# nessex/rdst

Measured on AMD Instinct MI355X. Metric: radix_sort_throughput_1B_uniform_u32, higher is better.
Workload: dtype u32; 1 GPU; 1000000000 uniform-random u32 keys per GPU, device-resident; route 'atomic': two MSD scatter passes that claim space with atomics (no counting read) + in-LDS sort of every bucket; keys_per_gpu=1000000000, total_keys=1000000000, seed=1565982722, route=atomic, parallelism=single

## Files before the change

### rdst_amd/csrc/rdst_kernels.hip

```cpp

#include <hip/hip_runtime.h>
#include <stdint.h>
#include <string.h>
#include <stdio.h>
#include <stdlib.h>
#include <stddef.h>
#include <mutex>
#include <type_traits>
#include <string>
#include <vector>
#include <map>
#include <utility>

#include "rdst_hip.h"
#include "rdst_internal.h"

namespace {

constexpr int RADIX = 256;
constexpr int MAX_LEVELS = 16;

constexpr uint32_t ST_EMPTY = 0, ST_AGG = 1, ST_INCL = 2;
template <typename S> struct StatusWord {
    static constexpr int SHIFT = sizeof(S) * 8 - 2;
// ... 1395 lines not shown
        if constexpr (STAGES > 1) {
            if (stage > 0) __syncthreads();
#pragma unroll
            for (int i = 0; i < KPT; ++i) {
                const uint32_t sl = (i & 1) ? (slots[i >> 1] >> 16) : (slots[i >> 1] & 0xFFFFu);
                const uint32_t rel = sl - (uint32_t)(stage * STAGE_KEYS);
                if (rel < (uint32_t)STAGE_KEYS) s_keys[rel] = mk[i];
            }
            __syncthreads();
        }
        constexpr int SUB = SPT % 6 == 0 ? 6 : (SPT % 4 == 0 ? 4 : (SPT < 6 ? SPT : 6));
#pragma unroll
        for (int i0 = 0; i0 < SPT; i0 += SUB) {
            K kk[SUB];
            D dd[SUB];
            V vv[HAS_V ? SUB : 1];
#pragma unroll
            for (int i = 0; i < SUB; ++i)
                if (i0 + i < SPT) kk[i] = s_keys[tid + (i0 + i) * BLOCK];
            if constexpr (HAS_V) {
#pragma unroll
                for (int i = 0; i < SUB; ++i)
                    if (i0 + i < SPT) vv[i] = s_vals[tid + (i0 + i) * BLOCK];
            }
#pragma unroll
            for (int i = 0; i < SUB; ++i)
                if (i0 + i < SPT) dd[i] = s_delta[digit_of(kk[i], shift)];
#pragma unroll
            for (int i = 0; i < SUB; ++i) {
                if (i0 + i >= SPT) continue;
                const uint32_t p = (uint32_t)(stage * STAGE_KEYS) + (uint32_t)tid + (uint32_t)(i0 + i) * BLOCK;
                K out = kk[i];
                if constexpr (MAPPED) out = unmap_key<K>(out, neg, pos);
                if (RDST_ABL(1) && out != (K)0x12345) continue;
                if (RDST_ABL(2)) {
                    if (full || p < valid) dst[tile_begin + p] = out;
                    continue;
                }
                if constexpr (NARROW) {
                    const uint32_t g = dd[i] + p * (uint32_t)sizeof(K);
                    const bool ok = g < (uint32_t)n * (uint32_t)sizeof(K);
                    bad |= !ok && (full || p < valid);
                    if constexpr (OUT16) {
                        if (halves) {
                            if (ok && (full || p < valid)) *reinterpret_cast<uint16_t*>(reinterpret_cast<unsigned char*>(out16) + (g >> 1)) = (uint16_t)kk[i];
                            continue;
                        }
                    }
                    if (ok && (full || p < valid)) {
                        *reinterpret_cast<K*>(reinterpret_cast<unsigned char*>(dst) + g) = out;
                        if constexpr (HAS_V) {
                            const uint32_t gv = sizeof(V) == sizeof(K) ? g : (sizeof(V) > sizeof(K) ? g * (uint32_t)(sizeof(V) / sizeof(K)) : g / (uint32_t)(sizeof(K) / sizeof(V)));
                            *reinterpret_cast<V*>(reinterpret_cast<unsigned char*>(vdst) + gv) = vv[i];
                        }
                    }
                } else {
                    const uint64_t g = dd[i] + p;
                    const bool ok = g < n;
                    bad |= !ok && (full || p < valid);
                    if (ok && (full || p < valid)) {
                        dst[g] = out;
                        if constexpr (HAS_V) vdst[g] = vv[i];
                    }
                }
            }
        }
    }
    if (bad) atomicOr(err, ERR_SCATTER_RANGE | ((uint32_t)(level + 1) << 8));
#ifdef RDST_EXPERIMENTS
    RDST_STAMP(9);
    if (tl_on) {
        uint32_t* rec = g_exp_timeline + (size_t)(chain_row0 + t) * 12;
        for (int k = 0; k < 10; ++k) rec[k] = tl[k];
        rec[10] = __builtin_amdgcn_s_getreg(20 | (0 << 6) | (3 << 11));
        rec[11] = blockIdx.x;
    }
#endif
    if constexpr (!PERSIST) break;
    __syncthreads();
    }
#undef RDST_ABL
}

struct MsdRanges {
    uint64_t start[CHAINS + 1];
};

template <typename K, int KPT, int NWAVES, bool MAPPED, bool SECOND, bool HALVES>
#ifndef RDST_MSD_MINWAVES
#define RDST_MSD_MINWAVES ((2 * NWAVES + 3) / 4)
#endif
__global__ __launch_bounds__(NWAVES * 64, RDST_MSD_MINWAVES) void msd_scatter_kernel(
    const K* __restrict__ src, const uint32_t* __restrict__ area_count , uint64_t n, uint32_t area_cap,
    uint32_t tiles_per_area, K* __restrict__ dst, uint16_t* __restrict__ dst16, uint32_t* __restrict__ cursor, uint32_t dst_cap, int shift,
    uint32_t slices ,
    const Plan* __restrict__ plan, uint32_t* __restrict__ overflow, uint32_t* __restrict__ inversion ,
    K neg, K pos,
    K* __restrict__ xbuf, K* __restrict__ xout, const uint32_t* __restrict__ bstart, const uint32_t* __restrict__ xtile0,
    MsdRanges xr) {
    static_assert(!HALVES || (SECOND && sizeof(K) == 4), "halves: the second pass of 4-byte keys");
    constexpr int BLOCK = NWAVES * 64, TILE = BLOCK * KPT;
    constexpr uint32_t SLOT_UNIT = (uint32_t)sizeof(K);
    const bool exact = plan->pre != 0;
    if (exact) {
        if (plan->route != ROUTE_HYBRID || plan->sorted_known) return;
        if (!SECOND && plan->pre_skip_a) return;
    } else {
        if (plan->gross_skew || plan->top_skew || plan->predict_lsd) return;
        if (SECOND && *inversion == 0) return;
    }
    const int win = exact ? 0 : (int)plan->win_shift;
    shift -= win;
    extern __shared__ __attribute__((aligned(16))) unsigned char smem[];
    uint32_t* wave_hist = reinterpret_cast<uint32_t*>(smem);
    uint32_t* s_delta = reinterpret_cast<uint32_t*>(smem + NWAVES * 1024);
    uint32_t* s_misc = reinterpret_cast<uint32_t*>(smem + NWAVES * 1024 + 1024);
    K* s_keys = reinterpret_cast<K*>(smem + NWAVES * 1024 + 1024 + 128);
    const int tid = threadIdx.x, lane = tid & 63, wave = tid >> 6;
    static_assert(NWAVES <= 16, "one word of s_misc per wave");
    uint32_t gave_up = 0;
    if (!exact) {
        gave_up = ld_relaxed<uint32_t>(overflow);
        if constexpr (!SECOND) {
            if (gave_up) {
                if (lane == 0) s_misc[16 + wave] = 1u;
                __syncthreads();
                return;
            }
        }
    }
    uint32_t area = blockIdx.x / tiles_per_area, j = blockIdx.x % tiles_per_area;
    if constexpr (SECOND) {
        if (!exact && slices == (uint32_t)CHAINS) {
            const uint32_t x = blockIdx.x % CHAINS, k = blockIdx.x / CHAINS;
            const uint32_t q = k / tiles_per_area;
            j = k % tiles_per_area;
            area = (q % CHAINS) * RADIX + (x + CHAINS * (q / CHAINS));
        }
        if (!exact && (blockIdx.x / tiles_per_area >= RADIX * slices || area >= RADIX * slices)) return;
    }
    uint64_t acount = area_count ? (uint64_t)area_count[area] : n;
    const K* asrc = src + (uint64_t)area * area_cap;
    if (exact) {
        if constexpr (!SECOND) {
            area = blockIdx.x % CHAINS; j = blockIdx.x / CHAINS;
            acount = xr.start[area + 1] - xr.start[area];
            asrc = src + xr.start[area];
        } else {
            if (blockIdx.x >= xtile0[RADIX]) return;
            uint32_t d = 0;
#pragma unroll
            for (int b = 7; b >= 0; --b) {
                const uint32_t c = d | (1u << b);
                if (xtile0[c] <= blockIdx.x) d = c;
            }
            area = d; j = blockIdx.x - xtile0[d];
            const uint32_t r0 = bstart[d * RADIX];
            acount = bstart[(d + 1) * RADIX] - r0;
            asrc = (plan->pre_skip_a ? static_cast<const K*>(xout) : static_cast<const K*>(xbuf)) + r0;
        }
    }
    const uint64_t tile_off = (uint64_t)j * TILE;
    if (tile_off >= acount) return;
    const uint32_t valid = acount - tile_off < (uint64_t)TILE ? (uint32_t)(acount - tile_off) : (uint32_t)TILE;
    const bool full = valid == (uint32_t)TILE;
    const K* tsrc = asrc + tile_off;
    RDST_TL_BEGIN(SECOND ? 3u : 2u);
    __builtin_amdgcn_s_setprio(RDST_PRIO_LOAD);
    K mk[KPT];
    const uint32_t wbase = (uint32_t)wave * 64u * KPT + (uint32_t)lane;
    K edge = 0;
    if constexpr (!SECOND) {
        if (lane == 0 && tile_off + (uint64_t)wave * 64u * KPT > 0 && (uint32_t)wave * 64u * KPT < valid) edge = tsrc[(int64_t)wbase - 1];
    }
    if (full) {
#pragma unroll
        for (int i = 0; i < KPT; ++i) mk[i] = tsrc[wbase + i * 64];
        if constexpr (MAPPED) {
#pragma unroll
            for (int i = 0; i < KPT; ++i) mk[i] = map_key<K>(mk[i], neg, pos);
        }
    } else {
#pragma unroll
        for (int i = 0; i < KPT; ++i) {
            const uint32_t idx = wbase + i * 64;
            K v = (K)~(K)0;
            if (idx < valid) {
                v = tsrc[idx];
                if constexpr (MAPPED) v = map_key<K>(v, neg, pos);
            }
            mk[i] = v;
        }
    }
    if constexpr (!SECOND) if (!exact) {
        if constexpr (MAPPED) edge = map_key<K>(edge, neg, pos);
        if (tile_off + (uint64_t)wave * 64u * KPT == 0) edge = 0;
        bool inv = false;
#pragma unroll
        for (int i = 0; i < KPT; ++i) {
            K before = lane_below<K>(mk[i]);
// ... 72 lines not shown
                        ranked = true;
                    }
                    run3[h] += (uint32_t)__builtin_popcountll(m);
                }
                if (!ranked) r = atomicAdd(&wh[d], 1u);
                if (i & 1) run_index[i >> 1] |= r << 16;
                else run_index[i >> 1] = r;
            }
#pragma unroll
            for (int h = 0; h < NHEAVY; ++h)
                if (lane == 0 && hd3[h] != 0xFFFFFFFFu) wh[hd3[h]] = run3[h];
        } else if (fast) {
#pragma unroll
            for (int i = 0; i < KPT; ++i) {
                const uint32_t r = atomicAdd(&wh[digit_of(mk[i], shift)], 1u);
                if (i & 1) run_index[i >> 1] |= r << 16;
                else run_index[i >> 1] = r;
            }
        } else {
#pragma unroll
            for (int i = 0; i < KPT; ++i) atomicAdd(&wh[digit_of(mk[i], shift)], 1u);
        }
    }
    RDST_STAMP(2);
    if (lane == 0) s_misc[16 + wave] = gave_up;
    __syncthreads();
    {
        uint32_t any = 0;
#pragma unroll
        for (int w = 0; w < NWAVES; ++w) any |= s_misc[16 + w];
        if (any) return;
    }
    RDST_STAMP(3);
    if (tid < RADIX) __builtin_amdgcn_s_setprio(RDST_PRIO_SCAN);
    uint32_t cw[NWAVES];
    uint32_t count_d = 0, pub = 0;
    if (tid < RADIX) {
#pragma unroll
        for (int w = 0; w < NWAVES; ++w) {
            cw[w] = wave_hist[w * RADIX + tid];
            count_d += cw[w];
        }
        pub = count_d;
        if (tid == RADIX - 1) pub -= (uint32_t)TILE - valid;
    }
    uint32_t incl = count_d;
#pragma unroll
    for (int o = 1; o < 64; o <<= 1) {
        const uint32_t y = __shfl_up(incl, o);
        if (lane >= o) incl += y;
    }
    if (tid < RADIX && lane == 63) s_misc[4 + wave] = incl;
    if (tid == 0) s_misc[1] = 0;
    __syncthreads();
    if (tid < RADIX) {
        uint32_t woff = 0;
        for (int w = 0; w < wave; ++w) woff += s_misc[4 + w];
        const uint32_t local_off = woff + incl - count_d;
        uint32_t run = local_off;
#pragma unroll
        for (int w = 0; w < NWAVES; ++w) {
            wave_hist[w * RADIX + tid] = run * SLOT_UNIT;
            run += cw[w];
        }
        const uint32_t where = SECOND ? (area % RADIX) * RADIX + (uint32_t)tid : (exact ? area : blockIdx.x % slices) * RADIX + (uint32_t)tid;
        uint32_t got = 0;
        if (pub) {
            got = atomicAdd(&cursor[where], pub);
            if (!exact && got + pub > dst_cap) {
                if (ld_relaxed<uint32_t>(overflow) == 0) atomicOr(overflow, 1u);
                s_misc[1] = 1;
            }
        }
        s_delta[tid] = (exact ? 0u : where * dst_cap) + got - local_off;
    }
    RDST_STAMP(4);
    __syncthreads();
    RDST_STAMP(5);
    __builtin_amdgcn_s_setprio(0);
    if (fast) {
#pragma unroll
        for (int i = 0; i < KPT; ++i) {
            const uint32_t idx = (i & 1) ? (run_index[i >> 1] >> 16) : (run_index[i >> 1] & 0xFFFFu);
            const uint32_t sl = wh[digit_of(mk[i], shift)] + idx * SLOT_UNIT;
            *reinterpret_cast<K*>(reinterpret_cast<unsigned char*>(s_keys) + sl) = mk[i];
        }
    } else if (!careful) {
#pragma unroll
        for (int i = 0; i < KPT; ++i) {
            uint32_t* slot = &wh[digit_of(mk[i], shift)];
            const uint32_t b = *slot;
            const uint32_t below = peers_below(digit_word<K>(mk[i], shift), bit0);
            __builtin_amdgcn_wave_barrier();
            atomicAdd(slot, SLOT_UNIT);
            *reinterpret_cast<K*>(reinterpret_cast<unsigned char*>(s_keys) + b + below * SLOT_UNIT) = mk[i];
        }
    } else {
#pragma unroll
        for (int i = 0; i < KPT; ++i) {
            uint32_t* slot = &wh[digit_of(mk[i], shift)];
            const uint32_t b = *slot;
            uint32_t below;
            if ((uniform_rounds >> i) & 1u) {
                below = (uint32_t)lane;
                __builtin_amdgcn_wave_barrier();
                if (lane == 0) *slot = b + 64u * SLOT_UNIT;
            } else {
                uint32_t total;
                below = peers_below_total(digit_word<K>(mk[i], shift), bit0, total);
                __builtin_amdgcn_wave_barrier();
                if (below == 0) *slot = b + total * SLOT_UNIT;
            }
            *reinterpret_cast<K*>(reinterpret_cast<unsigned char*>(s_keys) + b + below * SLOT_UNIT) = mk[i];
        }
    }
    RDST_STAMP(6);
    __syncthreads();
    RDST_STAMP(7);
    if (s_misc[1]) return;
    __builtin_amdgcn_s_setprio(RDST_PRIO_SCATTER);
    constexpr int SUB = KPT % 6 == 0 ? 6 : (KPT % 4 == 0 ? 4 : (KPT < 6 ? KPT : 6));
#pragma unroll
    for (int i0 = 0; i0 < KPT; i0 += SUB) {
        K kk[SUB];
        uint32_t dd[SUB];
#pragma unroll
        for (int i = 0; i < SUB; ++i)
            if (i0 + i < KPT) kk[i] = s_keys[tid + (i0 + i) * BLOCK];
#pragma unroll
        for (int i = 0; i < SUB; ++i)
            if (i0 + i < KPT) dd[i] = s_delta[digit_of(kk[i], shift)];
#pragma unroll
        for (int i = 0; i < SUB; ++i) {
            if (i0 + i >= KPT) continue;
            const uint32_t p = (uint32_t)tid + (uint32_t)(i0 + i) * BLOCK;
            if (full || p < valid) {
                const uint32_t g = dd[i] + p;
                if constexpr (HALVES) dst16[g] = (uint16_t)kk[i];
                else (exact ? (SECOND ? xout : xbuf) : dst)[g] = MAPPED ? unmap_key<K>(kk[i], neg, pos) : kk[i];
            }
        }
    }
    RDST_STAMP(8);
    RDST_TL_END(blockIdx.x);
}

constexpr int SMALL_WAVES = 16;
constexpr int SMALL_THREADS = SMALL_WAVES * 64;
constexpr int small_kpt(size_t key_bytes) { return key_bytes <= 4 ? 16 : (key_bytes == 8 ? 8 : 4); }

template <typename K, int LEVELS, bool MAPPED>
__global__ __launch_bounds__(SMALL_THREADS) void small_sort_kernel(K* __restrict__ keys, uint32_t n, K neg, K pos) {
    constexpr int KPT = small_kpt(sizeof(K));
    constexpr int TILE = SMALL_THREADS * KPT;
    extern __shared__ __attribute__((aligned(16))) unsigned char smem[];
    uint32_t* wave_hist = reinterpret_cast<uint32_t*>(smem);
    uint32_t* s_sum = reinterpret_cast<uint32_t*>(smem + SMALL_WAVES * 1024);
    K* stage = reinterpret_cast<K*>(smem + SMALL_WAVES * 1024 + 16);
    const int tid = threadIdx.x, lane = tid & 63, wave = tid >> 6;
    const int rounds = (int)((n + SMALL_THREADS - 1) / SMALL_THREADS);
    const uint32_t live = (uint32_t)rounds * SMALL_THREADS;
    const uint32_t wbase = (uint32_t)wave * 64u * (uint32_t)rounds + (uint32_t)lane;
    K mk[KPT];
#pragma unroll
    for (int i = 0; i < KPT; ++i) {
        const uint32_t idx = wbase + i * 64;
        K v = (K) ~(K)0;
        if (i < rounds && idx < n) {
            v = keys[idx];
            if constexpr (MAPPED) v = map_key<K>(v, neg, pos);
        }
        mk[i] = v;
    }
    uint32_t* wh = wave_hist + wave * RADIX;
    for (int level = 0; level < LEVELS; ++level) {
        const int shift = level * 8, bit0 = shift & 31;
#pragma unroll
        for (int j = 0; j < 4; ++j) wh[lane + 64 * j] = 0;
#pragma unroll
        for (int i = 0; i < KPT; ++i)
            if (i < rounds) atomicAdd(&wh[digit_of(mk[i], shift)], 1u);
        __syncthreads();
        uint32_t cw[SMALL_WAVES], count_d = 0;
        if (tid < RADIX) {
#pragma unroll
            for (int w = 0; w < SMALL_WAVES; ++w) { cw[w] = wave_hist[w * RADIX + tid]; count_d += cw[w]; }
        }
        const bool trivial = __syncthreads_or(tid < RADIX && count_d == live) != 0;
        if (trivial) continue;
        uint32_t incl = count_d;
#pragma unroll
        for (int o = 1; o < 64; o <<= 1) {
            const uint32_t y = __shfl_up(incl, o);
            if (lane >= o) incl += y;
        }
        if (tid < RADIX && lane == 63) s_sum[wave] = incl;
        __syncthreads();
        if (tid < RADIX) {
            uint32_t run = incl - count_d;
            for (int w = 0; w < wave; ++w) run += s_sum[w];
#pragma unroll
            for (int w = 0; w < SMALL_WAVES; ++w) { wave_hist[w * RADIX + tid] = run; run += cw[w]; }
        }
        __syncthreads();
#pragma unroll
        for (int i = 0; i < KPT; ++i) {
            if (i < rounds) {
                uint32_t* slot = &wh[digit_of(mk[i], shift)];
                const uint32_t b = *slot;
                const uint32_t below = peers_below(digit_word<K>(mk[i], shift), bit0);
                __builtin_amdgcn_wave_barrier();
                atomicAdd(slot, 1u);
                stage[b + below] = mk[i];
            }
// ... 243 lines not shown
        local_sort_bucket<K, NWAVES, KPT, MAPPED>(buf, src16, alt_src, slot_count ? bucket * slot_cap : start, bucket, bucket_prefix16(plan, bucket), start, cnt, err, neg, pos, flags);
        __syncthreads();
    }
}

constexpr int COUNT_TILE = local_tile(4);
constexpr size_t count_lds_bytes() { return 32768 + 16384 + 128; }
static_assert(2 * ((size_t)COUNT_TILE + 4) <= 32768 + 16384, "the output staging (shifted by up to three keys) aliases the counter and prefix tables");

__device__ __forceinline__ uint32_t nibble_sum(uint32_t x, uint32_t acc) {
    const uint32_t t = (x & 0x0F0F0F0Fu) + ((x >> 4) & 0x0F0F0F0Fu);
    return __builtin_amdgcn_sad_u8(t, 0u, acc);
}

constexpr int COUNT_SAFE = 24;

template <int BLOCK, bool MAPPED, bool FROM16, bool FAST, bool VEC>
__device__ __forceinline__ void count_sort_bucket(uint32_t* __restrict__ buf, const uint16_t* __restrict__ src16, uint32_t soff, uint32_t start, uint32_t cnt,
                                                  uint32_t bucket, const Plan* __restrict__ plan, uint32_t neg, uint32_t pos, uint32_t* __restrict__ list,
                                                  uint32_t* __restrict__ list_count, unsigned char* smem) {
    constexpr int MAXR = (COUNT_TILE + BLOCK - 1) / BLOCK;
    constexpr int VPT = H16_BINS / BLOCK, WPT = VPT / 8;
    constexpr int LOG_VPT = BLOCK == 1024 ? 6 : (BLOCK == 512 ? 7 : 8);
    static_assert((1 << LOG_VPT) == VPT, "block size");
    static_assert(!VEC || (FROM16 && MAXR == 33 && BLOCK == 512), "vector loads: four vectors of eight halves and one half per thread");
    static_assert(COUNT_SAFE % 8 == 0 && COUNT_SAFE < MAXR, "whole vectors");
    const int tid = threadIdx.x, lane = tid & 63, wave = tid >> 6;
    uint32_t* cnt4 = reinterpret_cast<uint32_t*>(smem);
    uint16_t* prefix = reinterpret_cast<uint16_t*>(smem + 32768);
    uint16_t* out16 = reinterpret_cast<uint16_t*>(smem);
    uint32_t* s_wsum = reinterpret_cast<uint32_t*>(smem + 32768 + 16384);
    auto idx_of = [&](int i) -> uint32_t {
        if constexpr (VEC) return i < 32 ? 8u * ((uint32_t)tid + (uint32_t)(i >> 3) * BLOCK) + (uint32_t)(i & 7) : 32u * BLOCK + (uint32_t)tid;
        else return (uint32_t)tid + (uint32_t)i * BLOCK;
    };
    uint32_t nvalid = 0;
    if constexpr (VEC) {
#pragma unroll
        for (int j = 0; j < 4; ++j) {
            const uint32_t v0 = 8u * ((uint32_t)tid + (uint32_t)j * BLOCK);
            nvalid += cnt > v0 ? (cnt - v0 < 8u ? cnt - v0 : 8u) : 0u;
        }
        nvalid += 32u * BLOCK + (uint32_t)tid < cnt ? 1u : 0u;
    } else {
        nvalid = cnt > (uint32_t)tid ? (cnt - (uint32_t)tid + BLOCK - 1u) / BLOCK : 0u;
    }
#define RDST_K4_PHASE() uint32_t nv_ = nvalid; asm volatile("" : "+v"(nv_))
#define RDST_K4_VALID(i) ((FAST && (i) < COUNT_SAFE) || (uint32_t)(i) < nv_)
#define RDST_K4_FENCE(i) do { if (((i) & 3) == 3 || (i) == MAXR - 1) { _Pragma("unroll") for (int f_ = (i) - ((i) & 3); f_ <= (i); ++f_) asm volatile("" : "+v"(kv[f_])); } } while (0)
#define RDST_K4_OPAQUE() do { _Pragma("unroll") for (int i_ = 0; i_ < MAXR; ++i_) asm volatile("" : "+v"(kv[i_])); } while (0)
    __builtin_amdgcn_s_setprio(RDST_PRIO_LOAD);
    uint32_t kv[MAXR];
    if constexpr (VEC) {
        const uint4* vsrc = reinterpret_cast<const uint4*>(src16 + soff);
        uint4 q[4];
#pragma unroll
        for (int j = 0; j < 4; ++j) {
            const uint32_t vi = (uint32_t)tid + j * BLOCK;
            if ((FAST && j < COUNT_SAFE / 8) || 8u * vi < cnt) q[j] = vsrc[vi];
            else q[j] = make_uint4(0, 0, 0, 0);
        }
        kv[32] = 32u * BLOCK + (uint32_t)tid < cnt ? (uint32_t)src16[soff + 32u * BLOCK + (uint32_t)tid] : 0u;
#pragma unroll
        for (int j = 0; j < 4; ++j) {
            const uint32_t d[4] = {q[j].x, q[j].y, q[j].z, q[j].w};
#pragma unroll
            for (int e = 0; e < 4; ++e) {
                kv[8 * j + 2 * e] = d[e] & 0xFFFFu;
                kv[8 * j + 2 * e + 1] = d[e] >> 16;
            }
        }
    } else {
        RDST_K4_PHASE();
#pragma unroll
        for (int i = 0; i < MAXR; ++i) {
            const uint32_t idx = idx_of(i);
            const uint32_t at = RDST_K4_VALID(i) ? idx : cnt - 1;
            if constexpr (FROM16) kv[i] = src16[soff + at];
            else kv[i] = buf[start + at];
        }
    }
#pragma unroll
    for (int k = 0; k < WPT; ++k) cnt4[k * BLOCK + tid] = 0;
    if (tid == 0) s_wsum[16] = 0;
    __syncthreads();
    __builtin_amdgcn_s_setprio(0);
    auto word_of = [](uint32_t v) -> uint32_t { return v >> 3; };
    bool over = false;
    {
    RDST_K4_PHASE();
#pragma unroll
    for (int i = 0; i < MAXR; ++i) {
        if (RDST_K4_VALID(i)) {
            const uint32_t v = FROM16 ? kv[i] : ((MAPPED ? map_key<uint32_t>(kv[i], neg, pos) : kv[i]) & 0xFFFFu);
            const uint32_t sh = (v & 7u) * 4u;
            const uint32_t old = atomicAdd(&cnt4[word_of(v)], 1u << sh);
            const uint32_t mine = (old >> sh) & 15u;
            over |= mine == 15u;
            kv[i] = v | (mine << 16);
        }
        RDST_K4_FENCE(i);
    }
    }
    if (over) s_wsum[16] = 1;
    __syncthreads();
    if (s_wsum[16]) {
        bool differ = false;
        uint32_t mine_first = 0;
        bool have = false;
        RDST_K4_PHASE();
#pragma unroll
        for (int i = 0; i < MAXR; ++i) {
            if (RDST_K4_VALID(i)) {
                if (!have) { mine_first = kv[i] & 0xFFFFu; have = true; }
                differ |= (kv[i] & 0xFFFFu) != mine_first;
            }
        }
        if (tid == 0) s_wsum[17] = mine_first;
        const int any = __syncthreads_or((int)differ);
        const bool agree = !have || mine_first == s_wsum[17];
        if (!any && !__syncthreads_or((int)!agree)) {
            const uint32_t m = (bucket_prefix16(plan, bucket) << 16) | s_wsum[17];
            const uint32_t out = MAPPED ? unmap_key<uint32_t>(m, neg, pos) : m;
            for (uint32_t idx = (uint32_t)tid; idx < cnt; idx += BLOCK) buf[start + idx] = out;
            return;
        }
        if (tid == 0) list[atomicAdd(list_count, 1u)] = bucket;
        return;
    }
    {
        constexpr int ROT_SHIFT = WPT == 16 ? 2 : 3;
        static_assert(WPT == 16 || WPT == 8, "64 banks / WPT lanes per rotation");
        const uint32_t r = ((uint32_t)tid >> ROT_SHIFT) & (uint32_t)(WPT - 1);
        uint32_t arr[WPT];
        uint32_t run = 0, through_last = 0;
#pragma unroll
        for (int k = 0; k < WPT; ++k) {
            const uint32_t j = ((uint32_t)k + r) & (uint32_t)(WPT - 1);
            arr[k] = run;
            run = nibble_sum(cnt4[WPT * tid + j], run);
            through_last = j == (uint32_t)(WPT - 1) ? run : through_last;
        }
        const uint32_t below_r = run - through_last;
        uint32_t incl = run;
#pragma unroll
        for (int o = 1; o < 64; o <<= 1) {
            const uint32_t y = __shfl_up(incl, o);
            if (lane >= o) incl += y;
        }
        if (lane == 63) s_wsum[wave] = incl;
        __syncthreads();
        uint32_t base = incl - run;
#pragma unroll
        for (int x = 0; x < BLOCK / 64; ++x)
            if (x < wave) base += s_wsum[x];
#pragma unroll
        for (int k = 0; k < WPT; ++k) {
            const uint32_t j = ((uint32_t)k + r) & (uint32_t)(WPT - 1);
            const uint32_t before = (uint32_t)k + r < (uint32_t)WPT ? below_r + arr[k] : arr[k] - through_last;
            prefix[WPT * tid + j] = (uint16_t)(base + before);
        }
    }
    __syncthreads();
    uint32_t* tdst = buf + start;
    const uint32_t mis = (uint32_t)(reinterpret_cast<uintptr_t>(tdst) >> 2) & 3u;
    {
    RDST_K4_PHASE();
    RDST_K4_OPAQUE();
#pragma unroll
    for (int i = 0; i < MAXR; ++i) {
        if (RDST_K4_VALID(i)) {
            const uint32_t v = kv[i] & 0xFFFFu, mine = kv[i] >> 16;
            const uint32_t wd = word_of(v);
            const uint32_t below = cnt4[wd] & ((1u << ((v & 7u) * 4u)) - 1u);
            const uint32_t slot = nibble_sum(below, (uint32_t)prefix[wd] + mine + mis);
            kv[i] = v | (slot << 16);
        }
        RDST_K4_FENCE(i);
    }
    }
    __syncthreads();
    {
    RDST_K4_PHASE();
    RDST_K4_OPAQUE();
#pragma unroll
    for (int i = 0; i < MAXR; ++i) {
        if (RDST_K4_VALID(i)) out16[kv[i] >> 16] = (uint16_t)kv[i];
    }
    }
    __syncthreads();
    __builtin_amdgcn_s_setprio(RDST_PRIO_SCATTER);
    const uint32_t top = bucket_prefix16(plan, bucket) << 16;
    const uint32_t quads = (cnt + mis + 3u) >> 2;
    constexpr int QR = (COUNT_TILE + 3 + 3) / 4 / BLOCK + 1;
    const uint2* o2 = reinterpret_cast<const uint2*>(out16);
    uint4* gq = reinterpret_cast<uint4*>(tdst - mis);
#pragma unroll
    for (int r = 0; r < QR; ++r) {
        const uint32_t qi = (uint32_t)tid + (uint32_t)r * BLOCK;
        if (qi < quads) {
            const uint2 h = o2[qi];
            uint4 k4;
            k4.x = top | (h.x & 0xFFFFu); k4.y = top | (h.x >> 16); k4.z = top | (h.y & 0xFFFFu); k4.w = top | (h.y >> 16);
            if constexpr (MAPPED) {
                k4.x = unmap_key<uint32_t>(k4.x, neg, pos); k4.y = unmap_key<uint32_t>(k4.y, neg, pos);
                k4.z = unmap_key<uint32_t>(k4.z, neg, pos); k4.w = unmap_key<uint32_t>(k4.w, neg, pos);
            }
            const uint32_t p0 = 4u * qi;
            if (p0 >= mis && p0 + 3u < mis + cnt) {
                gq[qi] = k4;
            } else {
                uint32_t* g = reinterpret_cast<uint32_t*>(gq + qi);
                if (p0 + 0u >= mis && p0 + 0u < mis + cnt) g[0] = k4.x;
                if (p0 + 1u >= mis && p0 + 1u < mis + cnt) g[1] = k4.y;
                if (p0 + 2u >= mis && p0 + 2u < mis + cnt) g[2] = k4.z;
                if (p0 + 3u >= mis && p0 + 3u < mis + cnt) g[3] = k4.w;
            }
        }
    }
}
#undef RDST_K4_PHASE
#undef RDST_K4_FENCE
#undef RDST_K4_OPAQUE
#undef RDST_K4_VALID

template <int BLOCK, bool MAPPED, bool FROM16>
__global__ __launch_bounds__(BLOCK, BLOCK == 1024 ? 8 : 6) void local_count_sort_kernel(
    uint32_t* __restrict__ buf_keys, uint32_t* __restrict__ buf_tmp, const uint16_t* __restrict__ src16, const uint32_t* __restrict__ bstart,
    const Plan* __restrict__ plan, uint32_t* __restrict__ err, uint32_t neg, uint32_t pos, uint32_t* __restrict__ list,
    uint32_t* __restrict__ list_count, const uint32_t* __restrict__ slot_count , uint32_t slot_cap) {
    if (!plan->local_sort) return;
    if (plan->route != ROUTE_ATOMIC) slot_count = nullptr;
    uint32_t* __restrict__ buf = plan->result_in_tmp ? buf_tmp : buf_keys;
    const uint32_t bucket = blockIdx.x;
    const uint32_t start = bstart[bucket], cnt = slot_count ? slot_count[bucket] : bstart[bucket + 1] - start;
    const uint32_t soff = slot_count ? bucket * slot_cap : start;
    const int tid = threadIdx.x;
    if (cnt <= 1) {
        if constexpr (FROM16) {
            if (cnt == 1 && tid == 0) {
                const uint32_t m = (bucket_prefix16(plan, bucket) << 16) | (uint32_t)src16[soff];
                buf[start] = MAPPED ? unmap_key<uint32_t>(m, neg, pos) : m;
            }
        }
        return;
    }
    if (cnt >= GIANT_MIN && plan->giants) return;
    if (cnt > (uint32_t)COUNT_TILE || plan->low_dups) {
        if (tid == 0) list[atomicAdd(list_count, 1u)] = bucket;
        return;
    }
    extern __shared__ __attribute__((aligned(16))) unsigned char smem[];
    const bool fast = cnt >= (uint32_t)COUNT_SAFE * BLOCK;
    if constexpr (FROM16 && BLOCK == 512) {
        if (slot_count) {
            if (fast) count_sort_bucket<BLOCK, MAPPED, FROM16, true, true>(buf, src16, soff, start, cnt, bucket, plan, neg, pos, list, list_count, smem);
            else count_sort_bucket<BLOCK, MAPPED, FROM16, false, true>(buf, src16, soff, start, cnt, bucket, plan, neg, pos, list, list_count, smem);
            return;
// ... 1378 lines not shown
    bool split = true;
    bool split_always = false;
    bool predict = true;
};
struct Tuning : RouteTuning {
    int pass_cfg = -1;
    int hist_bpc = 0;
    bool profiling = false;
    bool chains = true;
    int fast_rank = 1;
    bool small_sort = true;
    bool persist_fallback = true;
    uint64_t hybrid_min_len = 0;
};
uint32_t g_ablate = 0;
#ifdef RDST_EXPERIMENTS
size_t g_exp_lds_total = 0;
#endif
Tuning g_tuning;

constexpr RouteTuning route_preset(bool atomic_route, bool RouteTuning::*field = nullptr, bool value = false) {
    RouteTuning r;
    r.atomic_route = atomic_route;
    if (field) r.*field = value;
    return r;
}
constexpr struct RouteMode { int mode; const char* name; RouteTuning preset; } kRouteModes[] = {
    {7, "k1h", route_preset(false)},
    {0, "lsd", route_preset(false, &RouteTuning::hybrid, false)},
    {1, "default", route_preset(true)},
    {2, "ranked", route_preset(false, &RouteTuning::count_sort, false)},
    {3, "count_whole_keys", route_preset(false, &RouteTuning::halves, false)},
    {5, "no_presample", route_preset(false, &RouteTuning::presample, false)},
    {6, "wide_one_block", route_preset(false, &RouteTuning::wide2, false)},
    {8, "atomic_4_only", route_preset(true, &RouteTuning::atomic_wide, false)},
    {9, "no_expand", route_preset(false, &RouteTuning::expand, false)},
    {10, "atomic_then_lsd", route_preset(true, &RouteTuning::chain_routes, false)},
    {11, "no_giants", route_preset(true, &RouteTuning::giants, false)},
    {12, "no_exact_msd", route_preset(true, &RouteTuning::exact_msd, false)},
    {14, "no_predict", route_preset(true, &RouteTuning::predict, false)},
    {15, "wide2", route_preset(true, &RouteTuning::wide3, false)},
    {16, "no_split", route_preset(true, &RouteTuning::split, false)},
    {17, "split_always", route_preset(true, &RouteTuning::split_always, true)},
};
std::mutex g_mutex;

struct DeviceState {
    bool init = false;
    int cus = 256;
    void* ws = nullptr;
    size_t ws_bytes = 0;
    uint32_t* host_err = nullptr;
    uint32_t* err_dev = nullptr;
    hipStream_t host_stream = nullptr;
    void* host_buf = nullptr;
    size_t host_buf_bytes = 0;
    std::mutex host_mutex;
    hipEvent_t host_ev[4] = {nullptr, nullptr, nullptr, nullptr};
    bool host_timed = false;
    hipEvent_t last_done = nullptr;
    hipStream_t last_stream = nullptr;
    bool have_last = false;
    bool last_plan_valid = false;
    size_t last_plan_off = 0;
    std::vector<hipEvent_t> prof_events;
    std::vector<uint32_t> prof_kinds;
    uint32_t prof_used = 0;
    struct ProfRun { uint32_t begin, count; };
    std::vector<ProfRun> prof_runs;
};
DeviceState g_dev[16];

#ifndef RDST_MSD_WAVES
#define RDST_MSD_WAVES 12
#endif
#ifndef RDST_MSD_KPT4
#define RDST_MSD_KPT4 22
#endif
#ifndef RDST_MSD_KPT8
#define RDST_MSD_KPT8 11
#endif
constexpr int MSD_WAVES = RDST_MSD_WAVES;
constexpr int msd_kpt(size_t key_bytes) { return key_bytes == 4 ? RDST_MSD_KPT4 : RDST_MSD_KPT8; }

struct Layout {
    uint32_t levels, tile, status_bytes;
    uint64_t tiles;
    size_t off_err, off_tickets, off_plan, off_hpos, off_hpair, off_h16, off_hpos16, off_status, off_status_near, zero_bytes, off_hist, off_base,
        off_cbase, off_chains, off_bstart, off_fblist, off_fblist2, off_xtile0, off_glist, off_gsplit, off_gtables, off_halves, off_cursor_a, off_cursor_b, off_msd_a, total;
    uint32_t msd_cap_a, msd_slices;
    uint32_t slot_cap;
};

size_t align_up(size_t x, size_t a) { return (x + a - 1) / a * a; }

int tile_keys(int cfg, uint32_t elem_bytes) {
    const PassCfg& p = kPassCfgs[cfg];
    return p.nwaves * 64 * kpt_for(p.kpt8, elem_bytes);
}

constexpr uint32_t GIANT_MAX = 4096;
static_assert(GIANT_MAX + 1 <= GIANT_ITEMS_LDS, "the giant kernels keep every giant's first work item in LDS");

Layout make_layout(uint64_t n, uint32_t elem_bytes, uint32_t levels, int cfg, uint32_t tile_override = 0, bool want_halves = false,
                   bool want_msd = false, bool want_giants = false) {
    Layout L{};
    L.levels = levels;
    L.tile = tile_override ? tile_override : (uint32_t)tile_keys(cfg, elem_bytes);
    L.tiles = n / L.tile + CHAINS + 2;
    L.status_bytes = n < (1ull << 30) ? 4 : 8;
    size_t o = 0;
    L.off_err = o; o += 64;
    o = align_up(o, 128);
    L.off_tickets = o; o += sizeof(uint32_t) * MAX_LEVELS * TICKET_ROW;
    L.off_plan = o; o += align_up(sizeof(Plan), 16);
    L.off_hpos = o; o += sizeof(uint64_t) * (size_t)levels * CHAINS * RADIX;
    L.off_hpair = o; o += sizeof(uint64_t) * (size_t)levels * CHAINS * RADIX;
    o = align_up(o, 128);
    L.off_cursor_a = o; o += sizeof(uint32_t) * RADIX * MSD_SLICES;
    L.off_cursor_b = o; o += sizeof(uint32_t) * (size_t)H16_BINS;
    L.off_h16 = o; o += sizeof(uint32_t) * (size_t)H16_BINS;
    L.off_hpos16 = o; o += sizeof(uint64_t) * 2 * (size_t)CHAINS * RADIX;
    L.off_status = o; o += (size_t)L.status_bytes * levels * L.tiles * RADIX;
    L.off_status_near = o; o += (size_t)L.status_bytes * levels * L.tiles * RADIX;
    L.zero_bytes = align_up(o, 16); o = L.zero_bytes;
    L.off_hist = o; o += sizeof(uint64_t) * (size_t)levels * RADIX;
    L.off_base = o; o += sizeof(uint64_t) * (size_t)levels * RADIX;
    L.off_cbase = o; o += sizeof(uint64_t) * (size_t)levels * CHAINS * RADIX;
    L.off_chains = o; o += sizeof(LevelChains) * (size_t)levels;
    o = align_up(o, 16);
    L.off_bstart = o; o += sizeof(uint32_t) * ((size_t)H16_BINS + 4);
    L.off_fblist = o; o += sizeof(uint32_t) * (size_t)H16_BINS;
    L.off_fblist2 = o; o += sizeof(uint32_t) * (size_t)H16_BINS;
    L.off_xtile0 = o; o += sizeof(uint32_t) * (RADIX + 8);
    L.off_glist = o; o += sizeof(uint32_t) * 3 * ((size_t)GIANT_MAX + 16);
    o = align_up(o, 32);
    L.off_gsplit = o;
    if (want_giants) o += sizeof(GiantItem) * (size_t)(n / GIANT_OUT + GIANT_MAX + 16);
    o = align_up(o, 256);
    L.off_halves = o;
    if (want_halves && !want_msd) o += align_up(sizeof(uint16_t) * n, 256);
    L.slot_cap = 0;
    if (want_msd) {
        const double mean = (double)n / H16_BINS;
        const uint64_t want = ((uint64_t)(mean + 10.0 * __builtin_sqrt(mean)) + 64 + 63) / 64 * 64;
        L.slot_cap = (uint32_t)(want < (uint64_t)local_tile(elem_bytes) ? want : (uint64_t)local_tile(elem_bytes));
        o += align_up((elem_bytes == 4 ? sizeof(uint16_t) : (size_t)elem_bytes) * H16_BINS * L.slot_cap, 256);
        if (o - L.off_halves < sizeof(uint16_t) * n) o = L.off_halves + align_up(sizeof(uint16_t) * n, 256);
    }
    L.off_msd_a = o;
    L.msd_cap_a = 0;
    L.msd_slices = 1;
    if (want_msd) {
        const uint64_t TILE = (uint64_t)MSD_WAVES * 64 * msd_kpt(elem_bytes);
        const uint64_t tiles = (n + TILE - 1) / TILE;
        L.msd_slices = tiles >= 64 * MSD_SLICES ? MSD_SLICES : 1;
        const double mean = (double)n / (RADIX * L.msd_slices);
#ifndef RDST_AREA_SLACK
#define RDST_AREA_SLACK 0.125
#endif
        const double slack = mean * RDST_AREA_SLACK > 8.0 * __builtin_sqrt(mean) ? mean * RDST_AREA_SLACK : 8.0 * __builtin_sqrt(mean);
        L.msd_cap_a = (uint32_t)(((uint64_t)(mean + slack) + 2 * TILE / RADIX + 64) / 64 * 64);
        o += align_up((size_t)elem_bytes * L.msd_cap_a * RADIX * L.msd_slices, 256);
    }
    L.off_gtables = L.off_msd_a;
    if (want_giants) {
// ... 424 lines not shown
        p.rp = pick_routes<LEVELS>(p, cfg, true);
        rc = ensure_workspace(*p.D, p.rp.L.total);
    }
    if (rc) return rc;
    p.w = WsView(static_cast<char*>(p.D->ws), p.rp.L);
    return workspace_acquire(*p.D, p.s);
}

template <int LEVELS, typename K, typename V>
int clear_workspace(Pipe<K, V>& p) {
    DeviceState& D = *p.D;
    const Layout& L = p.w.L;
    char* ws = p.w.ws;
    hipStream_t s = p.s;
    int rc;
    if (g_tuning.profiling) D.prof_runs.push_back({D.prof_used, 0});
    if ((rc = prof_mark(D, s))) return rc;
    const size_t level_rows = (size_t)L.status_bytes * L.tiles * RADIX;
    if (p.rp.try_atomic) {
        HIP_TRY(hipMemsetAsync(ws, 0, L.off_status, s));
    } else if (p.rp.try_hybrid && LEVELS > 2) {
        HIP_TRY(hipMemsetAsync(ws, 0, L.off_status, s));
        HIP_TRY(hipMemsetAsync(ws + L.off_status + level_rows * (LEVELS - 2), 0, level_rows * 2, s));
        HIP_TRY(hipMemsetAsync(ws + L.off_status_near + level_rows * (LEVELS - 2), 0, level_rows * 2, s));
    } else if (p.level_lo == 0 && p.level_hi == (uint32_t)LEVELS) {
        HIP_TRY(hipMemsetAsync(ws, 0, L.zero_bytes, s));
    } else {
        const size_t status_lo = L.off_status + level_rows * p.level_lo, status_hi = L.off_status + level_rows * p.level_hi;
        HIP_TRY(hipMemsetAsync(ws, 0, L.off_status, s));
        if (status_hi > status_lo) {
            HIP_TRY(hipMemsetAsync(ws + status_lo, 0, status_hi - status_lo, s));
            HIP_TRY(hipMemsetAsync(ws + status_lo + (L.off_status_near - L.off_status), 0, status_hi - status_lo, s));
        }
    }
    return prof_mark(D, s, RDST_STAGE_CLEAR);
}

template <typename K, typename V>
int clear_unless_hybrid(const Pipe<K, V>& p, uint32_t levels, uint32_t unless_atomic) {
    const uint64_t vecs = (uint64_t)p.w.L.status_bytes * p.w.L.tiles * RADIX * levels / 16;
    return launch("clear_unless_hybrid_kernel", clear_unless_hybrid_kernel, dim3((uint32_t)p.D->cus * 4), dim3(256), 0, p.s, p.w.plan,
                  p.w.template status<uint4>(), vecs, p.w.template status_near<uint4>(), vecs, unless_atomic);
}

template <typename K>
uint32_t hist_blocks(uint64_t n, int cus) {
    uint64_t blocks = (uint64_t)(g_tuning.hist_bpc > 0 ? g_tuning.hist_bpc : 1) * cus;
    const uint64_t per_block_min = (uint64_t)HIST_THREADS * (16 / sizeof(K)) * 4;
    const uint64_t max_useful = (n + per_block_min - 1) / per_block_min;
    if (blocks > max_useful) blocks = max_useful;
    uint64_t balanced = 1;
    while (balanced * balanced * 4096 < n * sizeof(K)) ++balanced;
    if (blocks > balanced) blocks = balanced;
    return (uint32_t)(blocks < 1 ? 1 : blocks);
}

template <int LEVELS, typename K, typename V>
int count_and_route(const Pipe<K, V>& p, uint32_t pre_launch, bool sample_first) {
    const WsView& w = p.w;
    int rc;
    if (sample_first)
        if ((rc = launch_presample(p))) return rc;
    if ((rc = launch_hist16(p, pre_launch))) return rc;
    if (!pre_launch)
        if ((rc = prof_mark(*p.D, p.s, RDST_STAGE_HIST16))) return rc;
    RouteArgs ra{};
    ra.h16 = w.h16;
    ra.hpos16 = w.hpos16;
    ra.overflow = w.h16_overflow;
    ra.inversion = w.inversion;
    ra.allow_skip = p.allow_skip ? 1u : 0u;
    ra.bstart = w.bstart;
    ra.hpos = w.hpos;
    ra.hpair = w.hpair;
    ra.plan = w.plan;
    ra.n = p.n;
    ra.levels = (uint32_t)LEVELS;
    ra.cap = sizeof(K) == 4 && g_tuning.count_sort && g_tuning.expand ? EXPAND_MAX : (uint32_t)local_tile(sizeof(K));
    ra.giant_max = p.rp.giants ? GIANT_MAX : 0u;
    ra.glist = w.glist;
    ra.gcount_item = w.gcount_item;
    ra.gexp_item = w.gexp_item;
    ra.pre_launch = pre_launch;
    ra.msd_tile = (uint32_t)(MSD_WAVES * 64 * msd_kpt(sizeof(K)));
    ra.cursor_a = w.cursor_a;
    ra.cursor_b = w.cursor_b;
    ra.xtile0 = w.xtile0;
    ra.skip_a_ok = sizeof(K) == 4 ? 1u : 0u;
    return launch("route_kernel", route_kernel, dim3(1), dim3(1024), 0, p.s, ra);
}

template <typename K>
uint32_t exact_ranges(const K* keys, uint64_t n, uint32_t blocks, uint64_t tile, MsdRanges* xr) {
    const uint64_t xpiece = hist_piece(n, blocks, (uint64_t)HIST_THREADS * vec_for<K>(aligned16(keys)) * 4);
    for (int r = 0; r <= CHAINS; ++r) {
        const uint64_t at = (uint64_t)hist_first_block((uint32_t)r, blocks) * xpiece;
        xr->start[r] = at < n ? at : n;
    }
    uint32_t tiles_x = 0;
    for (int r = 0; r < CHAINS; ++r) {
        const uint32_t t = (uint32_t)((xr->start[r + 1] - xr->start[r] + tile - 1) / tile);
        if (t > tiles_x) tiles_x = t;
    }
    return tiles_x * CHAINS;
}

template <int LEVELS, typename K, typename V>
int atomic_stage(const Pipe<K, V>& p) {
    constexpr int KPT = msd_kpt(sizeof(K)), NW = MSD_WAVES, TILE = NW * 64 * KPT, W = (int)sizeof(K) * 8;
    constexpr bool HALF = sizeof(K) == 4;
    constexpr size_t mlds = (size_t)NW * 1024 + 1024 + 128 + sizeof(K) * TILE;
    const WsView& w = p.w;
    const Layout& L = w.L;
    DeviceState& D = *p.D;
    hipStream_t s = p.s;
    K* area_a = w.template area_a<K>();
    uint16_t* slots16 = HALF ? w.slots16() : nullptr;
    K* slots = HALF ? nullptr : w.template slots<K>();
    int rc;
    if ((rc = launch_presample(p))) return rc;
    if (p.rp.try_hybrid && g_tuning.exact_msd)
        if ((rc = count_and_route<LEVELS>(p, 1u, false))) return rc;
    if ((rc = prof_mark(D, s, RDST_STAGE_SAMPLE))) return rc;
    MsdRanges xr{};
    const uint32_t tiles_x = exact_ranges(p.keys, p.n, p.blocks, TILE, &xr);
    const uint32_t tiles_a = (uint32_t)((p.n + TILE - 1) / TILE);
    const uint32_t tpa = (L.msd_cap_a + TILE - 1) / TILE;
    const uint32_t grid_a = tiles_a > tiles_x ? tiles_a : tiles_x;
    rc = with_bools([&](auto MAPPED) {
        return launch("msd_scatter_kernel (pass A)", msd_scatter_kernel<K, KPT, NW, MAPPED, false, false>, dim3(grid_a), dim3(NW * 64), mlds, s, p.keys,
                      nullptr, p.n, 0u, grid_a, area_a, nullptr, w.cursor_a, L.msd_cap_a, W - 8, L.msd_slices, w.plan, w.msd_overflow, w.inversion,
                      (K)p.km.neg, (K)p.km.pos, p.tmp, p.keys, w.bstart, w.xtile0, xr);
    }, p.mapped);
    if (rc) return rc;
    if ((rc = prof_mark(D, s, RDST_STAGE_MSD_A))) return rc;
    uint32_t grid_b = (uint32_t)RADIX * L.msd_slices * tpa;
    if (grid_b < tiles_a + RADIX) grid_b = tiles_a + RADIX;
    rc = with_bools([&](auto MAPPED) {
        return launch("msd_scatter_kernel (pass B)", msd_scatter_kernel<K, KPT, NW, MAPPED, true, HALF>, dim3(grid_b), dim3(NW * 64), mlds, s, area_a,
                      w.cursor_a, 0ull, L.msd_cap_a, tpa, slots, slots16, w.cursor_b, L.slot_cap, W - 16, L.msd_slices, w.plan, w.msd_overflow,
                      w.inversion, (K)p.km.neg, (K)p.km.pos, p.tmp, p.keys, w.bstart, w.xtile0, xr);
    }, p.mapped);
    if (rc) return rc;
    if ((rc = prof_mark(D, s, RDST_STAGE_MSD_B))) return rc;
    MsdFinishArgs fa{};
    fa.cursor_b = w.cursor_b;
    fa.overflow = w.msd_overflow;
    fa.inversion = w.inversion;
    fa.bstart = w.bstart;
    fa.plan = w.plan;
    fa.n = p.n;
    fa.allow_skip = p.allow_skip ? 1u : 0u;
    if ((rc = launch("msd_finish_kernel", msd_finish_kernel, dim3(1), dim3(1024), 0, s, fa))) return rc;
    if ((rc = prof_mark(D, s, RDST_STAGE_ROUTE))) return rc;
    if (!p.rp.try_hybrid) return clear_unless_hybrid(p, LEVELS, 0u);
    return RDST_OK;
}

template <int LEVELS, typename K, typename V>
int hybrid_stage(const Pipe<K, V>& p) {
    int rc;
    if ((rc = count_and_route<LEVELS>(p, 0u, !p.rp.try_atomic))) return rc;
    if (p.rp.try_atomic) rc = clear_unless_hybrid(p, LEVELS, 1u);
    else if (LEVELS > 2) rc = clear_unless_hybrid(p, LEVELS - 2, 0u);
    if (rc) return rc;
    return prof_mark(*p.D, p.s, RDST_STAGE_ROUTE);
}

template <int LEVELS, typename K, typename V>
int count_and_scan(const Pipe<K, V>& p) {
    const WsView& w = p.w;
    const bool routed = p.rp.try_hybrid || p.rp.try_atomic;
    uint64_t piece = 0;
    int rc;
    if (LEVELS > 1 && p.level_hi == p.level_lo + 1) rc = launch_hist<1>(p, false, nullptr, &piece, (int)p.level_lo);
    else rc = launch_hist<LEVELS>(p, p.pair, routed ? w.plan : nullptr, &piece);
    if (rc) return rc;
    if ((rc = prof_mark(*p.D, p.s, RDST_STAGE_HIST))) return rc;
    ScanArgs sa{};
    sa.hpos = w.hpos;
    sa.hpair = p.pair ? w.hpair : nullptr;
    sa.hist = w.hist;
    sa.base = w.base;
    sa.cbase = w.cbase();
    sa.chains = w.chains();
    sa.plan = w.plan;
    sa.tickets = w.tickets();
    sa.inversion = w.inversion;
    sa.n = p.n;
    sa.hist_piece = piece;
    sa.levels = (uint32_t)LEVELS;
    sa.allow_skip = p.allow_skip ? 1u : 0u;
    sa.level_lo = p.level_lo;
    sa.level_hi = p.level_hi;
    sa.hist_grid = p.blocks;
    sa.tile = w.L.tile;
    sa.use_chains = g_tuning.chains ? 1u : 0u;
    sa.halves = p.rp.halves ? 1u : 0u;
    sa.deliver_tmp = p.deliver_tmp ? 1u : 0u;
    if ((rc = launch("scan_kernel", scan_kernel, dim3(1), dim3(256 * SCAN_GROUPS), 0, p.s, sa))) return rc;
    return prof_mark(*p.D, p.s, RDST_STAGE_SCAN);
}

template <int LEVELS, typename K, typename V>
int pass_loop(const Pipe<K, V>& p) {
    for (uint32_t level = p.level_lo; level < p.level_hi; ++level) {
        int rc;
        if constexpr (ValBytes<V>::value != 0) rc = launch_pass_pairs(p, (int)level);
        else rc = launch_pass(p, (int)level, p.rp.halves && level + 1 == (uint32_t)LEVELS ? p.w.halves16() : nullptr, p.rp.try_atomic && g_tuning.persist_fallback);
        if (rc) return rc;
        if ((rc = prof_mark(*p.D, p.s, RDST_STAGE_PASS | (level << 8)))) return rc;
    }
    return RDST_OK;
}

template <typename T>
int launch_copyback(T* dst, const T* src, uint64_t n, const Plan* plan, uint32_t deliver_tmp, int cus, hipStream_t s) {
    uint64_t blocks = (n * sizeof(T) / 16 + 255) / 256;
    if (blocks > (uint64_t)cus * 16) blocks = (uint64_t)cus * 16;
    if (blocks < 1) blocks = 1;
    return with_bools([&](auto ALIGNED) {
        return launch("copyback_kernel", copyback_kernel<T, vec_for<T>(ALIGNED)>, dim3((uint32_t)blocks), dim3(256), 0, s, dst, src, n, plan, deliver_tmp);
// ... 1003 lines not shown
```

Baseline: 242.3 Gkeys/s.

## Stage low halves plus digit byte in pass-B LDS and retune its tile shape

In the second MSD pass for 4-byte keys, the LDS staging buffer now stores a 16-bit low half and an 8-bit digit per key instead of the whole 32-bit key. This cuts per-key LDS from 4 to 3 bytes and avoids recomputing the digit on readback. Pass B gets its own waves-per-block, keys-per-thread and launch bounds so more waves fit per CU, with matching tile and grid changes in the host and route code. Separately, the in-LDS bucket sort gains a fast path: when every nibble count stays below 16, it turns the count words into in-place exclusive prefixes with a multiply, so each key's rank becomes a shift-and-mask instead of a nibble_sum. The misalignment offset is folded into the prefix array.

Result: no change. 241.6 Gkeys/s (-0.3%).

```diff
diff --git a/rdst_amd/csrc/rdst_kernels.hip b/rdst_amd/csrc/rdst_kernels.hip
--- a/rdst_amd/csrc/rdst_kernels.hip
+++ b/rdst_amd/csrc/rdst_kernels.hip
@@ -1501,13 +1501,18 @@
 #undef RDST_ABL
 }
 
+constexpr size_t msd_lds_bytes(int nwaves, int kpt, size_t staged_bytes) { return (size_t)nwaves * 1024 + 1024 + 128 + staged_bytes * nwaves * 64 * kpt; }
+constexpr int msd_blocks_per_cu(int nwaves, int kpt, bool halves) {
+    const int by_lds = (int)(160 * 1024 / msd_lds_bytes(nwaves, kpt, halves ? 3 : 4)), by_waves = 32 / nwaves;
+    return by_lds < by_waves ? by_lds : by_waves;
+}
 struct MsdRanges {
     uint64_t start[CHAINS + 1];
 };
 
 template <typename K, int KPT, int NWAVES, bool MAPPED, bool SECOND, bool HALVES>
 #ifndef RDST_MSD_MINWAVES
-#define RDST_MSD_MINWAVES ((2 * NWAVES + 3) / 4)
+#define RDST_MSD_MINWAVES (((HALVES ? msd_blocks_per_cu(NWAVES, KPT, true) : 2) * NWAVES + 3) / 4)
 #endif
 __global__ __launch_bounds__(NWAVES * 64, RDST_MSD_MINWAVES) void msd_scatter_kernel(
     const K* __restrict__ src, const uint32_t* __restrict__ area_count , uint64_t n, uint32_t area_cap,
@@ -1519,7 +1524,7 @@
     MsdRanges xr) {
     static_assert(!HALVES || (SECOND && sizeof(K) == 4), "halves: the second pass of 4-byte keys");
     constexpr int BLOCK = NWAVES * 64, TILE = BLOCK * KPT;
-    constexpr uint32_t SLOT_UNIT = (uint32_t)sizeof(K);
+    constexpr uint32_t SLOT_UNIT = HALVES ? 1u : (uint32_t)sizeof(K);
     const bool exact = plan->pre != 0;
     if (exact) {
         if (plan->route != ROUTE_HYBRID || plan->sorted_known) return;
@@ -1535,6 +1540,12 @@
     uint32_t* s_delta = reinterpret_cast<uint32_t*>(smem + NWAVES * 1024);
     uint32_t* s_misc = reinterpret_cast<uint32_t*>(smem + NWAVES * 1024 + 1024);
     K* s_keys = reinterpret_cast<K*>(smem + NWAVES * 1024 + 1024 + 128);
+    uint16_t* s_low = reinterpret_cast<uint16_t*>(smem + NWAVES * 1024 + 1024 + 128);
+    uint8_t* s_digit = reinterpret_cast<uint8_t*>(s_low + TILE);
+    auto stage = [&](uint32_t at, K key, uint32_t d) {
+        if constexpr (HALVES) { s_low[at] = (uint16_t)key; s_digit[at] = (uint8_t)d; }
+        else *reinterpret_cast<K*>(reinterpret_cast<unsigned char*>(s_keys) + at) = key;
+    };
     const int tid = threadIdx.x, lane = tid & 63, wave = tid >> 6;
     static_assert(NWAVES <= 16, "one word of s_misc per wave");
     uint32_t gave_up = 0;
@@ -1773,23 +1784,25 @@
 #pragma unroll
         for (int i = 0; i < KPT; ++i) {
             const uint32_t idx = (i & 1) ? (run_index[i >> 1] >> 16) : (run_index[i >> 1] & 0xFFFFu);
-            const uint32_t sl = wh[digit_of(mk[i], shift)] + idx * SLOT_UNIT;
-            *reinterpret_cast<K*>(reinterpret_cast<unsigned char*>(s_keys) + sl) = mk[i];
+            const uint32_t d = digit_of(mk[i], shift);
+            stage(wh[d] + idx * SLOT_UNIT, mk[i], d);
         }
     } else if (!careful) {
 #pragma unroll
         for (int i = 0; i < KPT; ++i) {
-            uint32_t* slot = &wh[digit_of(mk[i], shift)];
+            const uint32_t d = digit_of(mk[i], shift);
+            uint32_t* slot = &wh[d];
             const uint32_t b = *slot;
             const uint32_t below = peers_below(digit_word<K>(mk[i], shift), bit0);
             __builtin_amdgcn_wave_barrier();
             atomicAdd(slot, SLOT_UNIT);
-            *reinterpret_cast<K*>(reinterpret_cast<unsigned char*>(s_keys) + b + below * SLOT_UNIT) = mk[i];
+            stage(b + below * SLOT_UNIT, mk[i], d);
         }
     } else {
 #pragma unroll
         for (int i = 0; i < KPT; ++i) {
-            uint32_t* slot = &wh[digit_of(mk[i], shift)];
+            const uint32_t d = digit_of(mk[i], shift);
+            uint32_t* slot = &wh[d];
             const uint32_t b = *slot;
             uint32_t below;
             if ((uniform_rounds >> i) & 1u) {
@@ -1802,7 +1815,7 @@
                 __builtin_amdgcn_wave_barrier();
                 if (below == 0) *slot = b + total * SLOT_UNIT;
             }
-            *reinterpret_cast<K*>(reinterpret_cast<unsigned char*>(s_keys) + b + below * SLOT_UNIT) = mk[i];
+            stage(b + below * SLOT_UNIT, mk[i], d);
         }
     }
     RDST_STAMP(6);
@@ -1816,11 +1829,14 @@
         K kk[SUB];
         uint32_t dd[SUB];
 #pragma unroll
+        for (int i = 0; i < SUB; ++i) {
+            if (i0 + i >= KPT) continue;
+            if constexpr (HALVES) { kk[i] = s_low[tid + (i0 + i) * BLOCK]; dd[i] = s_digit[tid + (i0 + i) * BLOCK]; }
+            else kk[i] = s_keys[tid + (i0 + i) * BLOCK];
+        }
+#pragma unroll
         for (int i = 0; i < SUB; ++i)
-            if (i0 + i < KPT) kk[i] = s_keys[tid + (i0 + i) * BLOCK];
-#pragma unroll
-        for (int i = 0; i < SUB; ++i)
-            if (i0 + i < KPT) dd[i] = s_delta[digit_of(kk[i], shift)];
+            if (i0 + i < KPT) dd[i] = s_delta[HALVES ? dd[i] : digit_of(kk[i], shift)];
 #pragma unroll
         for (int i = 0; i < SUB; ++i) {
             if (i0 + i >= KPT) continue;
@@ -2230,7 +2246,7 @@
     }
 #pragma unroll
     for (int k = 0; k < WPT; ++k) cnt4[k * BLOCK + tid] = 0;
-    if (tid == 0) s_wsum[16] = 0;
+    if (tid == 0) { s_wsum[16] = 0; s_wsum[18] = 0; }
     __syncthreads();
     __builtin_amdgcn_s_setprio(0);
     auto word_of = [](uint32_t v) -> uint32_t { return v >> 3; };
@@ -2276,19 +2292,24 @@
         if (tid == 0) list[atomicAdd(list_count, 1u)] = bucket;
         return;
     }
+    uint32_t* tdst = buf + start;
+    const uint32_t mis = (uint32_t)(reinterpret_cast<uintptr_t>(tdst) >> 2) & 3u;
+    bool wide;
     {
         constexpr int ROT_SHIFT = WPT == 16 ? 2 : 3;
         static_assert(WPT == 16 || WPT == 8, "64 banks / WPT lanes per rotation");
         const uint32_t r = ((uint32_t)tid >> ROT_SHIFT) & (uint32_t)(WPT - 1);
         uint32_t arr[WPT];
-        uint32_t run = 0, through_last = 0;
+        uint32_t run = 0, through_last = 0, wmax = 0;
 #pragma unroll
         for (int k = 0; k < WPT; ++k) {
             const uint32_t j = ((uint32_t)k + r) & (uint32_t)(WPT - 1);
             arr[k] = run;
             run = nibble_sum(cnt4[WPT * tid + j], run);
+            wmax = run - arr[k] > wmax ? run - arr[k] : wmax;
             through_last = j == (uint32_t)(WPT - 1) ? run : through_last;
         }
+        if (wmax > 15u) s_wsum[18] = 1;
         const uint32_t below_r = run - through_last;
         uint32_t incl = run;
 #pragma unroll
@@ -2306,13 +2327,33 @@
         for (int k = 0; k < WPT; ++k) {
             const uint32_t j = ((uint32_t)k + r) & (uint32_t)(WPT - 1);
             const uint32_t before = (uint32_t)k + r < (uint32_t)WPT ? below_r + arr[k] : arr[k] - through_last;
-            prefix[WPT * tid + j] = (uint16_t)(base + before);
+            prefix[WPT * tid + j] = (uint16_t)(base + before + mis);
+        }
+        wide = __builtin_amdgcn_readfirstlane((int)s_wsum[18]) != 0;
+        if (!wide) {
+#pragma unroll
+            for (int k = 0; k < WPT; ++k) {
+                cnt4[k * BLOCK + tid] *= 0x11111110u;
+                if ((k & 3) == 3) asm volatile("" ::: "memory");
+            }
         }
     }
     __syncthreads();
-    uint32_t* tdst = buf + start;
-    const uint32_t mis = (uint32_t)(reinterpret_cast<uintptr_t>(tdst) >> 2) & 3u;
-    {
+    if (!wide) {
+    RDST_K4_PHASE();
+    RDST_K4_OPAQUE();
+#pragma unroll
+    for (int i = 0; i < MAXR; ++i) {
+        if (RDST_K4_VALID(i)) {
+            const uint32_t v = kv[i] & 0xFFFFu, mine = kv[i] >> 16;
+            const uint32_t wd = word_of(v);
+            const uint32_t below = (cnt4[wd] >> ((v & 7u) * 4u)) & 15u;
+            const uint32_t slot = (uint32_t)prefix[wd] + below + mine;
+            kv[i] = v | (slot << 16);
+        }
+        RDST_K4_FENCE(i);
+    }
+    } else {
     RDST_K4_PHASE();
     RDST_K4_OPAQUE();
 #pragma unroll
@@ -2321,7 +2362,7 @@
             const uint32_t v = kv[i] & 0xFFFFu, mine = kv[i] >> 16;
             const uint32_t wd = word_of(v);
             const uint32_t below = cnt4[wd] & ((1u << ((v & 7u) * 4u)) - 1u);
-            const uint32_t slot = nibble_sum(below, (uint32_t)prefix[wd] + mine + mis);
+            const uint32_t slot = nibble_sum(below, (uint32_t)prefix[wd] + mine);
             kv[i] = v | (slot << 16);
         }
         RDST_K4_FENCE(i);
@@ -3866,6 +3907,14 @@
 #endif
 constexpr int MSD_WAVES = RDST_MSD_WAVES;
 constexpr int msd_kpt(size_t key_bytes) { return key_bytes == 4 ? RDST_MSD_KPT4 : RDST_MSD_KPT8; }
+#ifndef RDST_MSD_KPT4B
+#define RDST_MSD_KPT4B 20
+#endif
+#ifndef RDST_MSD_WAVES4B
+#define RDST_MSD_WAVES4B 8
+#endif
+constexpr int msd_kpt_b(size_t key_bytes) { return key_bytes == 4 ? RDST_MSD_KPT4B : msd_kpt(key_bytes); }
+constexpr int msd_waves_b(size_t key_bytes) { return key_bytes == 4 ? RDST_MSD_WAVES4B : MSD_WAVES; }
 
 struct Layout {
     uint32_t levels, tile, status_bytes;
@@ -4456,7 +4505,7 @@
     ra.gcount_item = w.gcount_item;
     ra.gexp_item = w.gexp_item;
     ra.pre_launch = pre_launch;
-    ra.msd_tile = (uint32_t)(MSD_WAVES * 64 * msd_kpt(sizeof(K)));
+    ra.msd_tile = (uint32_t)(msd_waves_b(sizeof(K)) * 64 * msd_kpt_b(sizeof(K)));
     ra.cursor_a = w.cursor_a;
     ra.cursor_b = w.cursor_b;
     ra.xtile0 = w.xtile0;
@@ -4484,6 +4533,9 @@
     constexpr int KPT = msd_kpt(sizeof(K)), NW = MSD_WAVES, TILE = NW * 64 * KPT, W = (int)sizeof(K) * 8;
     constexpr bool HALF = sizeof(K) == 4;
     constexpr size_t mlds = (size_t)NW * 1024 + 1024 + 128 + sizeof(K) * TILE;
+    constexpr int KPT_B = msd_kpt_b(sizeof(K)), NW_B = msd_waves_b(sizeof(K)), TILE_B = NW_B * 64 * KPT_B;
+    constexpr size_t mlds_b = msd_lds_bytes(NW_B, KPT_B, HALF ? 3 : sizeof(K));
+    static_assert(!HALF || msd_blocks_per_cu(NW_B, KPT_B, true) * NW_B > 2 * NW, "the halves form: more waves per CU than two blocks of whole keys");
     const WsView& w = p.w;
     const Layout& L = w.L;
     DeviceState& D = *p.D;
@@ -4499,7 +4551,7 @@
     MsdRanges xr{};
     const uint32_t tiles_x = exact_ranges(p.keys, p.n, p.blocks, TILE, &xr);
     const uint32_t tiles_a = (uint32_t)((p.n + TILE - 1) / TILE);
-    const uint32_t tpa = (L.msd_cap_a + TILE - 1) / TILE;
+    const uint32_t tpa = (L.msd_cap_a + TILE_B - 1) / TILE_B;
     const uint32_t grid_a = tiles_a > tiles_x ? tiles_a : tiles_x;
     rc = with_bools([&](auto MAPPED) {
         return launch("msd_scatter_kernel (pass A)", msd_scatter_kernel<K, KPT, NW, MAPPED, false, false>, dim3(grid_a), dim3(NW * 64), mlds, s, p.keys,
@@ -4509,9 +4561,10 @@
     if (rc) return rc;
     if ((rc = prof_mark(D, s, RDST_STAGE_MSD_A))) return rc;
     uint32_t grid_b = (uint32_t)RADIX * L.msd_slices * tpa;
-    if (grid_b < tiles_a + RADIX) grid_b = tiles_a + RADIX;
+    const uint32_t tiles_b = (uint32_t)((p.n + TILE_B - 1) / TILE_B);
+    if (grid_b < tiles_b + RADIX) grid_b = tiles_b + RADIX;
     rc = with_bools([&](auto MAPPED) {
-        return launch("msd_scatter_kernel (pass B)", msd_scatter_kernel<K, KPT, NW, MAPPED, true, HALF>, dim3(grid_b), dim3(NW * 64), mlds, s, area_a,
+        return launch("msd_scatter_kernel (pass B)", msd_scatter_kernel<K, KPT_B, NW_B, MAPPED, true, HALF>, dim3(grid_b), dim3(NW_B * 64), mlds_b, s, area_a,
                       w.cursor_a, 0ull, L.msd_cap_a, tpa, slots, slots16, w.cursor_b, L.slot_cap, W - 16, L.msd_slices, w.plan, w.msd_overflow,
                       w.inversion, (K)p.km.neg, (K)p.km.pos, p.tmp, p.keys, w.bstart, w.xtile0, xr);
     }, p.mapped);
```
